# VinAIResearch/Counting-DETR

Hardware: AMD Instinct MI355X
Metric: images/sec FSCD-147 2nd-stage train step (higher is better)
Workload: dtype forward bf16x3 (fp32 operands split hi+lo, 3 bf16 MFMAs per product); data / weight gradients bf16 (both operands rounded to bf16, 1 MFMA per product); fp32 accumulate, fp32 storage, fp32 attention softmax / norms / losses / optimizer; 1 GPU; FSCD-147 2nd-stage train step (ResNet-50-DC5 + RCDA enc6/dec6, Q=300 learned, 800x800, T=[37, 120]), fwd+matcher+loss+bwd+clip+AdamW; images_per_gpu=2, global_batch=2, parallelism=dp1, graph=True, precision=bf16x3, precision_backward=bf16, frozen_stage_prefetch=True

## Files before the change

### counting_detr_amd/_ffi.py

```python
import ctypes as C
import os

import torch

_HERE = os.path.dirname(os.path.abspath(__file__))
LIB_PATH = os.environ.get("CDETR_LIB") or os.path.join(_HERE, "lib", "libcdetr_hip.so")

ROWS_DENSE, ROWS_CONV_FWD, ROWS_CONV_DGRAD = 0, 1, 2
_p = C.c_void_p


class ConvGeom(C.Structure):
    _fields_ = [("mode", C.c_int32), ("Ha", C.c_int32), ("Wa", C.c_int32), ("Hc", C.c_int32), ("Wc", C.c_int32),
                ("kh", C.c_int32), ("kw", C.c_int32), ("stride", C.c_int32), ("pad", C.c_int32), ("dil", C.c_int32)]


class GemmDesc(C.Structure):
    _fields_ = [("M", C.c_int32), ("N", C.c_int32), ("K", C.c_int32), ("taps", C.c_int32), ("batch", C.c_int32),
                ("b_layout", C.c_int32), ("relu", C.c_int32), ("precision", C.c_int32), ("out_scale", C.c_float),
                ("A", _p), ("lda", C.c_int64), ("sA", C.c_int64),
                ("B", _p), ("ldb", C.c_int64), ("sB", C.c_int64),
                ("C", _p), ("ldc", C.c_int64), ("sC", C.c_int64),
                ("w_scale", _p), ("bias", _p), ("resid", _p), ("ldr", C.c_int64), ("gate", _p), ("ldg", C.c_int64),
                ("g", ConvGeom), ("B_split", _p), ("batch_inner", C.c_int32), ("flags", C.c_int32),
# ... 1 lines not shown
                ("splitk_ws", _p), ("splitk_ws_bytes", C.c_int64), ("A16lo", _p), ("B16", _p), ("gate16", _p), ("C16lo", _p)]


class WgradDesc(C.Structure):
    _fields_ = [("P", C.c_int32), ("Nout", C.c_int32), ("Cin", C.c_int32), ("taps", C.c_int32), ("batch", C.c_int32), ("precision", C.c_int32),
                ("dY", _p), ("ldy", C.c_int64), ("sY", C.c_int64),
                ("X", _p), ("ldx", C.c_int64), ("sX", C.c_int64),
                ("dW", _p), ("ldw", C.c_int64), ("sW", C.c_int64),
                ("w_scale", _p), ("dbias", _p), ("g", ConvGeom), ("batch_inner", C.c_int32), ("wg_target", C.c_int32),
                ("sY2", C.c_int64), ("sX2", C.c_int64), ("sW2", C.c_int64), ("dY16", _p), ("X16", _p)]


class RcdaFwdDesc(C.Structure):
    _fields_ = [("N", C.c_int32), ("L", C.c_int32), ("H", C.c_int32), ("W", C.c_int32), ("nh", C.c_int32),
                ("precision", C.c_int32), ("scale", C.c_float), ("q_row", _p), ("q_col", _p), ("k_row", _p), ("k_col", _p), ("v", _p),
                ("mask_row", _p), ("mask_col", _p), ("out", _p), ("a_row", _p), ("a_col", _p), ("ws", _p), ("ws_bytes", C.c_int64)]


class RcdaBwdDesc(C.Structure):
    _fields_ = [("N", C.c_int32), ("L", C.c_int32), ("H", C.c_int32), ("W", C.c_int32), ("nh", C.c_int32),
                ("precision", C.c_int32), ("scale", C.c_float), ("d_out", _p), ("a_row", _p), ("a_col", _p), ("v", _p),
                ("ds_row", _p), ("ds_col", _p), ("d_v", _p), ("k_row", _p), ("k_col", _p), ("dq_row", _p), ("dq_col", _p),
                ("q_row", _p), ("q_col", _p), ("dk_row", _p), ("dk_col", _p)]


class AttnDesc(C.Structure):
    _fields_ = [("q", _p), ("k", _p), ("v", _p), ("ldq", C.c_int64), ("ldk", C.c_int64), ("ldv", C.c_int64), ("o", _p), ("lse", _p),
                ("d_o", _p), ("d_q", _p), ("d_k", _p), ("d_v", _p), ("ld_dq", C.c_int64), ("ld_dk", C.c_int64), ("ld_dv", C.c_int64),
                ("work", _p), ("N", C.c_int32), ("Lq", C.c_int32), ("Lk", C.c_int32), ("nh", C.c_int32), ("scale", C.c_float),
                ("precision", C.c_int32)]

# ... 208 lines not shown
```

### counting_detr_amd/csrc/common.h

```cpp
#pragma once
#include <hip/hip_runtime.h>
#include <stdint.h>

typedef float f32x16 __attribute__((ext_vector_type(16)));
typedef float f32x4 __attribute__((ext_vector_type(4)));
typedef __bf16 bf16x8 __attribute__((ext_vector_type(8)));

#define CDETR_OK 0
#define CDETR_ERR_ARG (-1)
#define CDETR_ERR_LAUNCH (-2)
#define CDETR_ERR_UNSUPPORTED (-3)

#include <stdlib.h>
static inline const char* cdetr_tune_env(const char* name) {
    static const bool tuning = getenv("CDETR_TUNING") != nullptr;
    return tuning ? getenv(name) : nullptr;
}

void cdetr_set_error(const char* fmt, ...);

#define CDETR_CHECK_ARG(cond, ...)          \
    do {                                    \
        if (!(cond)) {                      \
            cdetr_set_error(__VA_ARGS__);   \
// ... 57 lines not shown

__device__ __forceinline__ void stash_split4(__bf16* dst, int lo_off, float x0, float x1, float x2, float x3) {
    uint2 h, l;
    split_bf16_pk(x0, x1, h.x, l.x);
    split_bf16_pk(x2, x3, h.y, l.y);
    *reinterpret_cast<uint2*>(dst) = h;
    *reinterpret_cast<uint2*>(dst + lo_off) = l;
}
__device__ __forceinline__ void stash_hi4(__bf16* dst, float x0, float x1, float x2, float x3) {
    const f32x2 v0 = {x0, x1}, v1 = {x2, x3};
    uint2 h;
    h.x = __builtin_bit_cast(unsigned, __builtin_convertvector(v0, bf16x2));
    h.y = __builtin_bit_cast(unsigned, __builtin_convertvector(v1, bf16x2));
    *reinterpret_cast<uint2*>(dst) = h;
}
__device__ __forceinline__ f32x16 mfma_bf16x3(const bf16x8& ah, const bf16x8& al, const bf16x8& bh, const bf16x8& bl, f32x16 acc) {
    acc = __builtin_amdgcn_mfma_f32_32x32x16_bf16(al, bh, acc, 0, 0, 0);
    acc = __builtin_amdgcn_mfma_f32_32x32x16_bf16(ah, bl, acc, 0, 0, 0);
    acc = __builtin_amdgcn_mfma_f32_32x32x16_bf16(ah, bh, acc, 0, 0, 0);
    return acc;
}

template <int TERMS>
__device__ __forceinline__ f32x16 mfma_bf16_terms(const bf16x8& ah, const bf16x8& al, const bf16x8& bh, const bf16x8& bl, f32x16 acc) {
    if constexpr (TERMS == 1) return __builtin_amdgcn_mfma_f32_32x32x16_bf16(ah, bh, acc, 0, 0, 0);
    else return mfma_bf16x3(ah, al, bh, bl, acc);
}

template <int CTRL, int ROW_MASK>
__device__ __forceinline__ float dpp_pull(float x, float fill) {
// ... 21 lines not shown
```

### counting_detr_amd/csrc/igemm.hip

```cpp
#include "../../include/cdetr_hip.h"
#include "common.h"
#include "rows.h"
#include <stdlib.h>
#include <type_traits>
#include <vector>
#include <algorithm>

namespace {

constexpr int BK = 16;
constexpr int LDS_K = BK + 4;

__device__ __forceinline__ float4 ld4(const float* p) { return *reinterpret_cast<const float4*>(p); }
typedef unsigned u32x4 __attribute__((ext_vector_type(4)));
__device__ __forceinline__ u32x4 ld16(const __bf16* p) { return *reinterpret_cast<const u32x4*>(p); }
__device__ __forceinline__ float4 zero4() { return make_float4(0.f, 0.f, 0.f, 0.f); }

template <int BM, int BN, int BL>
__global__ __launch_bounds__(256) void igemm_kernel(const cdetr_gemm_desc d, const int tilesM, const int vecA,
                                                    const int vecB) {
    constexpr int FM = BM / 64, FN = BN / 64;
    constexpr int A_SLOTS = BM / 64, B_SLOTS = BN / 64;
    constexpr int LDS_N = BN + 4;
    constexpr int B_TILE = (BL == 0) ? BN * LDS_K : BK * LDS_N;
// ... 187 lines not shown
            for (int r = 0; r < 16; ++r) { rv[r] = 0.f; gv[r] = 1.f; }
            if (d.resid) {
#pragma unroll
                for (int r = 0; r < 16; ++r) rv[r] = d.resid[(long)min(mbase + (r & 3) + 8 * (r >> 2), d.M - 1) * d.ldr + nc];
            }
            if (d.gate) {
#pragma unroll
                for (int r = 0; r < 16; ++r) gv[r] = d.gate[(long)min(mbase + (r & 3) + 8 * (r >> 2), d.M - 1) * d.ldg + nc];
            }
#pragma unroll
            for (int r = 0; r < 16; ++r) {
                const int m = mbase + (r & 3) + 8 * (r >> 2);
                float v = (acc[a][b][r] + bias) * d.out_scale + rv[r];
                v = gv[r] > 0.f ? v : 0.f;
                if (d.relu) v = fmaxf(v, 0.f);
                if (nvalid && m < d.M) { C[(long)m * d.ldc + n] = v; if (C16) C16[(long)m * d.ldc + n] = (__bf16)v; }
            }
        }
    }
}

template <int BI, int BJ>
__global__ __launch_bounds__(256) void wgrad_kernel(const cdetr_wgrad_desc d, const int tilesI, const int tilesJ,
                                                    const int kt_per_slice) {
    constexpr int FM = BI / 64, FN = BJ / 64;
    constexpr int A_SLOTS = BI / 64, B_SLOTS = BJ / 64;
    constexpr int LDI = BI + 4, LDJ = BJ + 4;
    __shared__ __attribute__((aligned(16))) float smem[2 * BK * LDI + 2 * BK * LDJ];
    float* As = smem;
    float* Bs = smem + 2 * BK * LDI;

// ... 804 lines not shown
        float* red = smem;
#pragma unroll
        for (int s = 0; s < A_SLOTS; ++s) *reinterpret_cast<float4*>(red + kr * BI + cq + 32 * s) = bsum[s];
        __syncthreads();
        for (int i = tid; i < BI; i += 256) {
            float t = 0.f;
#pragma unroll 8
            for (int r = 0; r < 32; ++r) t += red[r * BI + i];
            if (i0 + i < d.Nout) atomicAdd(dbias + i0 + i, t);
        }
    }
}



typedef short s16x4 __attribute__((ext_vector_type(4)));
typedef short s16x8 __attribute__((ext_vector_type(8)));
__device__ __forceinline__ bf16x8 lds_tr8(const __bf16* p0, const __bf16* p1) {
    const s16x4 a = __builtin_amdgcn_ds_read_tr16_b64_v4i16((__attribute__((address_space(3))) s16x4*)(p0));
    const s16x4 b = __builtin_amdgcn_ds_read_tr16_b64_v4i16((__attribute__((address_space(3))) s16x4*)(p1));
    const s16x8 c = __builtin_shufflevector(a, b, 0, 1, 2, 3, 4, 5, 6, 7);
    return __builtin_bit_cast(bf16x8, c);
}

template <int BI, int BJ, int TERMS = 3>
__device__ __forceinline__ void wgrad_tr_body(const cdetr_wgrad_desc& d, const int tilesI, const int tilesJ, const int kt_per_slice,
                                              float* __restrict__ dbias, const int bx, const int by, const int bz, const bool single) {
    constexpr int BKF = 32;
    constexpr int FM = BI / 64, FN = BJ / 64;
    constexpr int A_SLOTS = BI / 32, B_SLOTS = BJ / 32;
    constexpr int BLK = 32 * 32;
    constexpr int PLANE_A = A_SLOTS * BLK, PLANE_B = B_SLOTS * BLK;
    constexpr int BUF = 2 * (PLANE_A + PLANE_B);
    extern __shared__ __attribute__((aligned(16))) float smem[];
    __bf16* Zs = reinterpret_cast<__bf16*>(smem);

    const int tid = threadIdx.x;
    const int lane = tid & 63, wid = tid >> 6;
// ... 507 lines not shown
#pragma unroll
    for (int r = 0; r < 4; ++r) red[wid][r * 64 + lane] = acc[r];
    __syncthreads();
    if (wid != 0) return;
    const int no = tn * 16 + i;
    if (no >= d.N) return;
#pragma unroll
    for (int r = 0; r < 4; ++r) {
        const int mo = tm * 16 + g4 * 4 + r;
        if (mo >= d.M) continue;
        const float sum = (red[0][r * 64 + lane] + red[1][r * 64 + lane]) + (red[2][r * 64 + lane] + red[3][r * 64 + lane]);
        float v = (sum + bias) * d.out_scale + rv[r];
        v = gv[r] > 0.f ? v : 0.f;
        if (d.relu) v = fmaxf(v, 0.f);
        C[(long)mo * d.ldc + no] = v;
        if (C16) C16[(long)mo * d.ldc + no] = (__bf16)v;
    }
}

template <int BL, int UB>
__global__ __launch_bounds__(256) void igemm_direct_kernel(const cdetr_gemm_desc d, const int tilesM, const int tilesN,
                                                           const int vecA, const int vecB) {
    igemm_direct_body<BL, UB>(d, tilesM, tilesN, vecA, vecB, blockIdx.x, blockIdx.z);
}

template <int BL, int UB>
__global__ __launch_bounds__(256) void igemm_direct_group_kernel(const GemmGroupArgs g) {
    int p = 0;
    while (p + 1 < g.n && (int)blockIdx.x >= g.blk0[p + 1]) ++p;
    const GemmGroupItem& it = g.it[p];
    const int lb = blockIdx.x - g.blk0[p];
// ... 760 lines not shown
```

### counting_detr_amd/csrc/rcda.hip

```cpp
#include "../../include/cdetr_hip.h"
#include "common.h"
#include <algorithm>
#include <type_traits>
#include <stdlib.h>

namespace {

__device__ __forceinline__ void xcd_slab(int& bx, int& by) {
    const int gx = gridDim.x, total = gx * gridDim.y;
    if (total & 7) return;
    const int lin = by * gx + bx;
    const int l2 = (lin & 7) * (total >> 3) + (lin >> 3);
    by = l2 / gx;
    bx = l2 - by * gx;
}


constexpr int D = 32;
constexpr int QW = 32;

__device__ __forceinline__ float4 ld4(const float* p) { return *reinterpret_cast<const float4*>(p); }

struct FwdSmem {
    int sw, sh;
// ... 400 lines not shown
        stamp(2 + side);
    }
    __syncthreads();
    stamp(4);

    {
        const int nq = min(QW, L - qbase);
        if (nq > 0 && save && d.a_row != nullptr) {
            save_rows(Srow, sm.sw, d.a_row + (((long)n * d.nh + head) * L + qbase) * Wp, nq, Wp, lane);
            save_rows(Scol, sm.sh, d.a_col + (((long)n * d.nh + head) * L + qbase) * Hp, nq, Hp, lane);
        }
    }
    stamp(5);
}

struct Fwd2Smem { int off_v, vts, total; };
__host__ __device__ inline Fwd2Smem fwd2_smem(const FwdSmem& sm, int H, int W, int KS) {
    Fwd2Smem s;
    s.off_v = sm.off_k;
    s.vts = 32 * KS + 8;
    const int vfloats = 2 * 32 * s.vts / 2;
    const int kfloats = (W + H) * KSTR;
    s.total = sm.off_k + (kfloats > vfloats ? kfloats : vfloats);
    return s;
}

template <int NW, int KS, int TH = 2, bool PROBE = false>
__global__ __launch_bounds__(64 * NW) void rcda_fwd2_kernel(const cdetr_rcda_fwd_desc d) {
    unsigned long long pt[5] = {0, 0, 0, 0, 0}, pacc[3] = {0, 0, 0};
    auto now = [&]() __attribute__((always_inline)) -> unsigned long long {
        if constexpr (PROBE) { const unsigned long long t = __builtin_amdgcn_s_memtime(); asm volatile("s_waitcnt lgkmcnt(0)" ::: "memory"); return t; }
        return 0ull;
    };
    pt[0] = now();
    constexpr int NT = 64 * NW, QB = QW * NW;
    constexpr int PD = 4;
    constexpr int NBLK = 16 * 4 * KS;
    constexpr int VB = (NBLK + NT - 1) / NT;
    constexpr int VTS = 32 * KS + 8;
    extern __shared__ __attribute__((aligned(16))) float smem[];
    const int H = d.H, W = d.W, L = d.L, E = d.nh * D;
    const FwdSmem sm = fwd_smem(H, W, NW);
    const int tid = threadIdx.x, lane = tid & 63, wid = tid >> 6;
// ... 61 lines not shown
    for (int s = 0; s < KS; ++s) {
        float x[8];
#pragma unroll
        for (int j = 0; j < 8; ++j) {
            const int w = 16 * s + 8 * g + j;
            x[j] = (w < W) ? Srow[i32 * sm.sw + w] : 0.f;
        }
        split_bf16x8(x, bh[s], bl[s]);
    }

    float outT[16];
#pragma unroll
    for (int r = 0; r < 16; ++r) outT[r] = 0.f;
    const f32x16 zero = {0.f, 0.f, 0.f, 0.f, 0.f, 0.f, 0.f, 0.f, 0.f, 0.f, 0.f, 0.f, 0.f, 0.f, 0.f, 0.f};

    vfetch(rv[0]); vfetch(rv[1]); vfetch(rv[2]); vfetch(rv[3]);
    vstash(rv[0], 0);
    __syncthreads();
    pt[2] = now();
    auto step = [&](auto U, int h) __attribute__((always_inline)) {
        constexpr int u = decltype(U)::value;
        const unsigned long long s0 = now();
        vfetch(rv[u]);
        const unsigned long long s1 = now();
        const float acolh = (h < he) ? Scol[i32 * sm.sh + h] : 0.f;
        const __bf16* vt = VT + (u & 1) * 32 * VTS + i32 * VTS + 8 * g;
        f32x16 T = zero;
#pragma unroll
        for (int s = 0; s < KS; ++s) {
            const bf16x8 ah = *reinterpret_cast<const bf16x8*>(vt + 16 * s);
// ... 5 lines not shown
        unsigned long long s2 = 0;
        if constexpr (PROBE) { asm volatile("" :: "v"(outT[0]), "v"(outT[15])); s2 = now(); }
        vstash(rv[(u + 1) % PD], (u + 1) & 1);
        const unsigned long long s3 = now();
        __syncthreads();
        if constexpr (PROBE) {
            const unsigned long long s4 = now();
            pacc[0] += s4 - s3; pacc[1] += s2 - s1; pacc[2] += (s1 - s0) + (s3 - s2);
        }
    };
    for (int h0 = hb; h0 < he; h0 += PD) {
        step(std::integral_constant<int, 0>{}, h0);
        step(std::integral_constant<int, 1>{}, h0 + 1);
        step(std::integral_constant<int, 2>{}, h0 + 2);
        step(std::integral_constant<int, 3>{}, h0 + 3);
    }
    pt[3] = now();
    if (hs > 1) {
        int* cnt = reinterpret_cast<int*>(d.ws);
        float* wsp = reinterpret_cast<float*>(cnt + RCDA_WS_COUNTERS);
        const int tile = blockIdx.y * gridDim.x + blockIdx.x;
        float* mine = wsp + ((long)tile * hs + hz) * 16 * NT + tid;
#pragma unroll
        for (int r = 0; r < 16; ++r) __hip_atomic_store(mine + r * NT, outT[r], __ATOMIC_RELAXED, __HIP_MEMORY_SCOPE_AGENT);
        __builtin_amdgcn_s_waitcnt(0);
        __syncthreads();
        int* flag = reinterpret_cast<int*>(smem + sm.off_k);
        if (tid == 0) {
            const int old = __hip_atomic_fetch_add(cnt + tile, 1, __ATOMIC_RELAXED, __HIP_MEMORY_SCOPE_AGENT);
            const int last = (old == hs - 1) ? 1 : 0;
// ... 849 lines not shown
}
inline int rcda_probe() {
    const char* p = cdetr_tune_env("CDETR_RCDA_PROBE");
    return p ? atoi(p) : 0;
}

}

extern "C" int cdetr_rcda_fwd(const cdetr_rcda_fwd_desc* dp, void* stream) {
    CDETR_CHECK_ARG(dp != nullptr, "cdetr_rcda_fwd: null descriptor");
    const cdetr_rcda_fwd_desc d = *dp;
    CDETR_CHECK_ARG(d.N > 0 && d.L > 0 && d.H > 0 && d.W > 0 && d.nh > 0, "cdetr_rcda_fwd: bad sizes");
    CDETR_CHECK_ARG(d.H <= 128 && d.W <= 1024, "cdetr_rcda_fwd: H must be <= 128 (got %d)", d.H);
    CDETR_CHECK_ARG(d.q_row && d.q_col && d.k_row && d.k_col && d.v && d.out, "cdetr_rcda_fwd: null pointer");
    CDETR_CHECK_ARG((d.a_row != nullptr) == (d.a_col != nullptr), "cdetr_rcda_fwd: a_row and a_col are saved together or not at all (both NULL: inference)");
    hipStream_t st = reinterpret_cast<hipStream_t>(stream);
    if (d.precision == 1 && d.W <= 96) {
        const int ks = (d.W + 15) / 16;
        auto go = [&](auto kern, int NWv, int KSv = 0, bool sliced = true) -> int {
            const FwdSmem sm = fwd_smem(d.H, d.W, NWv);
            const int bytes = fwd2_smem(sm, d.H, d.W, KSv ? KSv : ks).total * 4;
            int rc;
            if ((rc = set_smem(kern, bytes, "cdetr_rcda_fwd"))) return rc;
            dim3 grid((d.L + QW * NWv - 1) / (QW * NWv), d.N * d.nh), block(64 * NWv);
            if (sliced) grid.z = fwd2_slices(d, (int)(grid.x * grid.y), 64 * NWv, bytes);
            hipLaunchKernelGGL(kern, grid, block, bytes, st, d);
            return cdetr_launch_status("cdetr_rcda_fwd");
        };
        if (const int probe = rcda_probe(); probe && d.ws && ks == 4 && d.H <= 64)
            return probe == 5 ? go(rcda_fwd2_kernel<5, 4, 2, true>, 5, 0, false) : go(rcda_fwd2_kernel<4, 4, 2, true>, 4, 0, false);
        if (ks == 4 && rcda_wg5(d.L, d.N * d.nh)) return go(rcda_fwd2_kernel<5, 4>, 5);
        if (ks > 4 || d.H > 64) {
            if (d.H > 64 && d.H <= 96) return ks <= 4 ? go(rcda_fwd2_kernel<4, 4, 3>, 4, 4) : go(rcda_fwd2_kernel<4, 6, 3>, 4, 6);
            if (ks <= 4) return go(rcda_fwd2_kernel<4, 4>, 4, 4);
            return ks == 5 ? go(rcda_fwd2_kernel<4, 5>, 4) : go(rcda_fwd2_kernel<4, 6>, 4);
        }
        if (ks == 1) return go(rcda_fwd2_kernel<4, 1>, 4);
        if (ks == 2) return go(rcda_fwd2_kernel<4, 2>, 4);
        if (ks == 3) return go(rcda_fwd2_kernel<4, 3>, 4);
        return go(rcda_fwd2_kernel<4, 4>, 4);
    }
    if (d.H <= 32) return launch_rcda_fwd<1>(d, st);
    if (d.H <= 64) return launch_rcda_fwd<2>(d, st);
    return launch_rcda_fwd<4>(d, st);
}
// ... 81 lines not shown
```

### counting_detr_amd/ops.py

```python
import os

import torch

from . import _ffi
from ._ffi import CriterionDesc, MirrorItem, ConvGeom, GemmDesc, RcdaBwdDesc, RcdaFwdDesc, WgradDesc, check, lib, ptr, stream_ptr

import ctypes as C


PROFILE = None

import os as _os
PRECISION = int(_os.environ.get("CDETR_PRECISION", "1"))
PRECISION_BWD = int(_os.environ.get("CDETR_PRECISION_BWD", "3"))
MHA_BWD_BF16 = _os.environ.get("CDETR_MHA_BWD_BF16", "0") == "1"


def bwd_precision():
    return PRECISION_BWD if PRECISION == 1 else PRECISION


class arithmetic:

    def __init__(self, precision, precision_bwd=None):
        self.want = (int(precision), int(PRECISION_BWD if precision_bwd is None else precision_bwd))

    def __enter__(self):
        global PRECISION, PRECISION_BWD
        self.saved = (PRECISION, PRECISION_BWD)
        PRECISION, PRECISION_BWD = self.want
        return self

    def __exit__(self, *exc):
        global PRECISION, PRECISION_BWD
        PRECISION, PRECISION_BWD = self.saved
        return False


class scope:
    _KEYS = ("MIRROR", "BRANCH_BESIDE", "WGRAD_EVERY", "AFTER_BACKBONE", "WG_DEFER_NESTED", "ZERO_ARENA", "RCDA_SAVE", "PROFILE")

    def __init__(self, **kw):
        assert all(k in self._KEYS for k in kw), kw
        self.want = kw

    def __enter__(self):
        g = globals()
        self.saved = {k: g[k] for k in self.want}
        g.update(self.want)
        return self

    def __exit__(self, *exc):
        globals().update(self.saved)
        return False

# ... 443 lines not shown
            return hit
        r = self._find(self.f_entries, self._fb, w, scale)
        if r is None:
            out = None
        else:
            (base, nbytes, off, R, Cc, taps, sptr, _), row0 = r
            out = self.flat_fs[off + row0 * Cc * taps:]
        self._memo_f[key] = out
        return out


AFTER_BACKBONE = None
MIRROR = None


def linear_fwd(x2d, weight, bias=None, relu=False, resid=None, out_scale=1.0, out=None):
    M, K = x2d.shape
    N = weight.shape[0]
    y = out if out is not None else torch.empty((M, N), device=x2d.device, dtype=torch.float32)
    sp = MIRROR.lookup_fwd(weight) if MIRROR is not None else None
    gemm_raw(x2d, x2d.stride(0), weight, weight.stride(0), y, y.stride(0), M, N, K, bias=bias, relu=relu,
             resid=resid, ldr=(resid.stride(0) if resid is not None else 0), out_scale=out_scale, B_split=sp)
    return y


def linear_dgrad(dy2d, weight, gate=None, resid=None, dy16=None, twin=False):
    M, N = dy2d.shape
    K = weight.shape[1]
    dx = torch.empty((M, K), device=dy2d.device, dtype=torch.float32)
    m = MIRROR.lookup(weight) if MIRROR is not None else None
    if m is not None:
        dx16 = torch.empty((M, K), device=dy2d.device, dtype=torch.bfloat16) if twin else None
        gemm_raw(dy2d, dy2d.stride(0), m[0], m[1], dx, K, M, K, N, b_layout=0,
                 gate=gate, ldg=(gate.stride(0) if gate is not None else 0),
                 resid=resid, ldr=(resid.stride(0) if resid is not None else 0), B_split=m[2], B16=m[3], precision=bwd_precision(),
                 A16=dy16, C16=dx16)
        return (dx, dx16) if twin else dx
    gemm_raw(dy2d, dy2d.stride(0), weight, weight.stride(0), dx, K, M, K, N, b_layout=1,
# ... 409 lines not shown
    Nb, H, W, Cc = x.shape
    Ho, Wo = (H - 1) // 2 + 1, (W - 1) // 2 + 1
    y = torch.empty((Nb, Ho, Wo, Cc), device=x.device, dtype=torch.float32)
    if split:
        yh = torch.empty((Nb, Ho, Wo, Cc), device=x.device, dtype=torch.bfloat16)
        yl = torch.empty((Nb, Ho, Wo, Cc), device=x.device, dtype=torch.bfloat16)
        check(lib().cdetr_maxpool3x3s2_split(ptr(x), ptr(y), ptr(yh), ptr(yl), Nb, H, W, Cc, stream_ptr()), "cdetr_maxpool3x3s2_split")
        return y, yh, yl
    check(lib().cdetr_maxpool3x3s2(ptr(x), ptr(y), Nb, H, W, Cc, stream_ptr()), "cdetr_maxpool3x3s2")
    return y


RCDA_SKIP_SAVE = os.environ.get("CDETR_RCDA_SKIP_SAVE", "1") != "0"
RCDA_SAVE = True
RCDA_SLICES = os.environ.get("CDETR_RCDA_SLICES", "1") != "0"
FUSE_RCDA_DQ = os.environ.get("CDETR_RCDA_FUSE_DQ", "1") != "0"
FUSE_RCDA_DK = os.environ.get("CDETR_RCDA_FUSE_DK", "1") != "0"


def rcda_pads(H, W):
    return (H + 7) & ~7, (W + 3) & ~3


def rcda_fwd_raw(q_row, q_col, k_row, k_col, v, mask_row, mask_col, nh, save=None):
    N, L, E = q_row.shape
    H, W = v.shape[1:3]
    assert E == nh * 32, "the RCDA kernels are specialised for head_dim 32"
    Hp, Wp = rcda_pads(H, W)
    if save is None:
        save = RCDA_SAVE or not RCDA_SKIP_SAVE
    out = torch.empty((N, L, E), device=v.device, dtype=torch.float32)
    a_row = torch.empty((N, nh, L, Wp), device=v.device, dtype=torch.float32) if save else None
    a_col = torch.empty((N, nh, L, Hp), device=v.device, dtype=torch.float32) if save else None
    d = RcdaFwdDesc()
    d.N, d.L, d.H, d.W, d.nh, d.scale = N, L, H, W, nh, 32 ** -0.5
    d.precision = PRECISION
    d.q_row, d.q_col, d.k_row, d.k_col, d.v = ptr(q_row), ptr(q_col), ptr(k_row), ptr(k_col), ptr(v)
    d.mask_row, d.mask_col = ptr(mask_row), ptr(mask_col)
    d.out, d.a_row, d.a_col = ptr(out), ptr(a_row), ptr(a_col)
    if RCDA_SLICES:
        d.ws, d.ws_bytes = ptr(splitk_ws()), SPLITK_BYTES
    fl = 2.0 * N * nh * L * (H * W * 32 + (H + W) * 32)
    with _Timed("rcda_fwd", fl, None,
                4.0 * N * (3 * L * E + (H + W) * E + H * W * E + nh * L * (Hp + Wp)), fl * _TERMS[d.precision]):
        check(lib().cdetr_rcda_fwd(C.byref(d), stream_ptr()), "cdetr_rcda_fwd")
    return out, a_row, a_col


def rcda_zero_numel(v, k_row, k_col):
    return v.numel() + k_row.numel() + k_col.numel()


def rcda_bwd_raw(d_out, q_row, q_col, k_row, k_col, v, a_row, a_col, nh, zbuf=None):
    N, L, E = q_row.shape
# ... 329 lines not shown
    N, H, W, Cc = T.shape
    out = torch.empty_like(T)
    check(lib().cdetr_bcast_add2(ptr(T), ptr(Br), ptr(Bc), ptr(out), N, H, W, Cc, sr, sc, stream_ptr()), "cdetr_bcast_add2")
    return out


def _wg(dy2d, x2d, wparam, bparam, lo, hi):
    if not wparam.requires_grad:
        return
    gw = grad_buffer(wparam)[lo:hi]
    gb = grad_buffer(bparam)[lo:hi] if (bparam is not None and bparam.requires_grad) else None
    wgrad_raw(dy2d, dy2d.stride(0), x2d, x2d.stride(0), gw, gw.stride(0), dy2d.shape[0], hi - lo, x2d.shape[1], dbias=gb,
              may_defer=True)


class EncoderLayerFn(torch.autograd.Function):

    @staticmethod
    def forward(ctx, src, posemb_row, posemb_col, mask_row, mask_col, layer, anchor):
        N, H, W, Cc = src.shape
        R = N * H * W
        att = layer.self_attn
        E, nh = att.embed_dim, att.num_heads
        Wi, bi = att.in_proj_weight.detach(), att.in_proj_bias.detach()
        X = src.contiguous()
        Prow, Pcol = posemb_row.contiguous(), posemb_col.contiguous()
        Qr, Qc, Kr, Kc = posadd2_hw_reduce(X, Prow, Pcol)
        with gemm_queue():
            q_row = linear_fwd(Qr.view(R, Cc), Wi[0:E], bi[0:E]).view(N, H * W, E)
            q_col = linear_fwd(Qc.view(R, Cc), Wi[E:2 * E], bi[E:2 * E]).view(N, H * W, E)
            k_row = linear_fwd(Kr.view(N * W, Cc), Wi[2 * E:3 * E], bi[2 * E:3 * E]).view(N, W, E)
            k_col = linear_fwd(Kc.view(N * H, Cc), Wi[3 * E:4 * E], bi[3 * E:4 * E]).view(N, H, E)
            v = linear_fwd(X.view(R, Cc), Wi[4 * E:5 * E], bi[4 * E:5 * E]).view(N, H, W, E)
        o, a_row, a_col = rcda_fwd_raw(q_row, q_col, k_row, k_col, v, mask_row, mask_col, nh)
        Y1 = linear_fwd(o.view(R, E), att.out_proj.weight.detach(), att.out_proj.bias.detach(), resid=X.view(R, Cc))
        X1, mu1, rs1 = ln_fwd_raw(Y1, layer.norm1.weight.detach(), layer.norm1.bias.detach(), layer.norm1.eps)
        f = layer.ffn
        Hd = linear_fwd(X1, f.linear1.weight.detach(), f.linear1.bias.detach(), relu=True)
        Y2 = linear_fwd(Hd, f.linear2.weight.detach(), f.linear2.bias.detach(), resid=X1)
        X2, mu2, rs2 = ln_fwd_raw(Y2, f.norm2.weight.detach(), f.norm2.bias.detach(), f.norm2.eps)
        ctx.save_for_backward(X, Qr, Qc, Kr, Kc, q_row, q_col, k_row, k_col, v, a_row, a_col, o, Y1, mu1, rs1, X1, Hd, Y2, mu2, rs2)
        ctx.layer, ctx.dims = layer, (N, H, W, Cc, E, nh)
        return X2.view(N, H, W, Cc)

    @staticmethod
    def backward(ctx, dX2):
        with wgrad_queue():
            return EncoderLayerFn._backward(ctx, dX2)

# ... 118 lines not shown
        mem2 = memory.view(N * H * W, E)
        ctx.own_means = krm is None
        if ctx.own_means:
            krm, kcm = hw_reduce(memory, memory, posemb_row.contiguous(), posemb_col.contiguous(), 1.0 / H, 1.0 / W)
        krm2, kcm2 = krm.contiguous().view(N * W, E), kcm.contiguous().view(N * H, E)
        outs = []
        saved = []
        x = tgt.view(M, E)
        mem_side = []
        with gemm_queue():
            for layer in layers:
                ca = layer.cross_attn
                Wc, bc = ca.in_proj_weight.detach(), ca.in_proj_bias.detach()
                mem_side.append((linear_fwd(krm2, Wc[2 * E:3 * E], bc[2 * E:3 * E]).view(N, W, E),
                                 linear_fwd(kcm2, Wc[3 * E:4 * E], bc[3 * E:4 * E]).view(N, H, E),
                                 linear_fwd(mem2, Wc[4 * E:5 * E], bc[4 * E:5 * E]).view(N, H, W, E)))
        a1_next = None
        for li, layer in enumerate(layers):
            sa, ca, f = layer.self_attn, layer.cross_attn, layer.ffn
            nh = sa.num_heads
            Ws, bs = sa.in_proj_weight.detach(), sa.in_proj_bias.detach()
            Wc, bc = ca.in_proj_weight.detach(), ca.in_proj_bias.detach()
            if a1_next is None:
                a1, _ = add2(x, qpos.view(M, E))
            else:
                a1 = a1_next
            with gemm_queue():
                qk = linear_fwd(a1, Ws[0:2 * E], bs[0:2 * E])
                vs = linear_fwd(x, Ws[2 * E:3 * E], bs[2 * E:3 * E])
            o1, lse = mha_fwd_raw(qk.view(N, L, 2 * E), vs.view(N, L, E), nh, lens)
            Y2 = linear_fwd(o1.view(M, E), sa.out_proj.weight.detach(), sa.out_proj.bias.detach(), resid=x)
            T1, mu2, rs2, qr_in, qc_in = ln_fwd_add_raw(Y2, layer.norm2.weight.detach(), layer.norm2.bias.detach(), layer.norm2.eps,
                                                        qx.view(M, E), qy.view(M, E))
            with gemm_queue():
                q_row = linear_fwd(qr_in, Wc[0:E], bc[0:E]).view(N, L, E)
                q_col = linear_fwd(qc_in, Wc[E:2 * E], bc[E:2 * E]).view(N, L, E)
            k_row, k_col, v = mem_side[li]
            o2, a_row, a_col = rcda_fwd_raw(q_row, q_col, k_row, k_col, v, mask_row, mask_col, ca.num_heads)
            Y1 = linear_fwd(o2.view(M, E), ca.out_proj.weight.detach(), ca.out_proj.bias.detach(), resid=T1)
            T2, mu1, rs1 = ln_fwd_raw(Y1, layer.norm1.weight.detach(), layer.norm1.bias.detach(), layer.norm1.eps)
            Hd = linear_fwd(T2, f.linear1.weight.detach(), f.linear1.bias.detach(), relu=True)
            Y3 = linear_fwd(Hd, f.linear2.weight.detach(), f.linear2.bias.detach(), resid=T2)
            if li + 1 < len(layers):
                out, mu3, rs3, a1_next, _ = ln_fwd_add_raw(Y3, f.norm2.weight.detach(), f.norm2.bias.detach(), f.norm2.eps, qpos.view(M, E))
            else:
                out, mu3, rs3 = ln_fwd_raw(Y3, f.norm2.weight.detach(), f.norm2.bias.detach(), f.norm2.eps)
            outs.append(out.view(N, L, E))
            saved.append((x, a1, qk, vs, o1, lse, Y2, mu2, rs2, T1, qr_in, qc_in, q_row, q_col, k_row, k_col, v, a_row, a_col, o2,
                          Y1, mu1, rs1, T2, Hd, Y3, mu3, rs3))
            x = out
        ctx.layers, ctx.saved, ctx.dims = layers, saved, (N, L, E, H, W)
        ctx.shared = (mem2, krm2, kcm2)
        ctx.set_materialize_grads(False)
# ... 601 lines not shown
```

### include/cdetr_hip.h

```cpp
#ifndef CDETR_HIP_H
#define CDETR_HIP_H
#include <stddef.h>
#include <stdint.h>

#ifdef __cplusplus
extern "C" {
#endif

#define CDETR_ABI_VERSION 2

#define CDETR_ROWS_DENSE 0
#define CDETR_ROWS_CONV_FWD 1
#define CDETR_ROWS_CONV_DGRAD 2

typedef struct {
    int32_t mode;
    int32_t Ha, Wa;
    int32_t Hc, Wc;
    int32_t kh, kw, stride, pad, dil;
} cdetr_conv_geom;

typedef struct {
    int32_t M, N, K, taps;
    int32_t batch;
// ... 114 lines not shown
int cdetr_weight_mirror(const cdetr_mirror_item* items_dev, int32_t n_items, int32_t total_tiles, void* stream);
int cdetr_weight_images(const cdetr_mirror_item* items_dev, int32_t n_items, int32_t total_blocks, void* stream);

int cdetr_maxpool3x3s2(const float* X, float* Y, int32_t Nimg, int32_t H, int32_t W, int32_t C, void* stream);
int cdetr_maxpool3x3s2_split(const float* X, float* Y, void* Y16, void* Y16lo, int32_t Nimg, int32_t H, int32_t W, int32_t C, void* stream);

typedef struct {
    int32_t N, L, H, W, nh;
    int32_t precision;
    float scale;
    const float* q_row; const float* q_col; const float* k_row; const float* k_col; const float* v;
    const uint8_t* mask_row; const uint8_t* mask_col;
    float* out; float* a_row; float* a_col;
    void* ws;
    int64_t ws_bytes;
} cdetr_rcda_fwd_desc;
int cdetr_rcda_fwd(const cdetr_rcda_fwd_desc* d, void* stream);

typedef struct {
    int32_t N, L, H, W, nh;
    int32_t precision;
    float scale;
    const float* d_out; const float* a_row; const float* a_col; const float* v;
    float* ds_row; float* ds_col; float* d_v;
    const float* k_row; const float* k_col;
    float* dq_row; float* dq_col;
    const float* q_row; const float* q_col;
    float* dk_row; float* dk_col;
} cdetr_rcda_bwd_desc;
int cdetr_rcda_bwd(const cdetr_rcda_bwd_desc* d, void* stream);
// ... 197 lines not shown
```

Before: 242.1 images/s.

## Emit bf16 hi/lo planes of V from projection epilogue and stream them in RCDA forward

The value-projection GEMM epilogue now also writes bf16 hi and lo planes of its output. The RCDA forward kernel gets a planes variant that streams those pre-split planes straight into LDS through a 4-deep global_load_lds ring, then reads them back with transposing LDS loads for the bf16x3 MFMAs. This removes the per-tile fp32 load, hi/lo split and register stash of V inside the attention kernel. The cost is two extra bf16 writes per V element in the GEMM, extra memory for the planes, and a larger shared-memory ring.

```diff
diff --git a/counting_detr_amd/_ffi.py b/counting_detr_amd/_ffi.py
--- a/counting_detr_amd/_ffi.py
+++ b/counting_detr_amd/_ffi.py
@@ -39,7 +39,8 @@
 class RcdaFwdDesc(C.Structure):
     _fields_ = [("N", C.c_int32), ("L", C.c_int32), ("H", C.c_int32), ("W", C.c_int32), ("nh", C.c_int32),
                 ("precision", C.c_int32), ("scale", C.c_float), ("q_row", _p), ("q_col", _p), ("k_row", _p), ("k_col", _p), ("v", _p),
-                ("mask_row", _p), ("mask_col", _p), ("out", _p), ("a_row", _p), ("a_col", _p), ("ws", _p), ("ws_bytes", C.c_int64)]
+                ("mask_row", _p), ("mask_col", _p), ("out", _p), ("a_row", _p), ("a_col", _p), ("ws", _p), ("ws_bytes", C.c_int64),
+                ("v16", _p), ("v16lo", _p)]
 
 
 class RcdaBwdDesc(C.Structure):
diff --git a/counting_detr_amd/csrc/common.h b/counting_detr_amd/csrc/common.h
--- a/counting_detr_amd/csrc/common.h
+++ b/counting_detr_amd/csrc/common.h
@@ -95,6 +95,14 @@
     h.y = __builtin_bit_cast(unsigned, __builtin_convertvector(v1, bf16x2));
     *reinterpret_cast<uint2*>(dst) = h;
 }
+typedef short s16x4 __attribute__((ext_vector_type(4)));
+typedef short s16x8 __attribute__((ext_vector_type(8)));
+__device__ __forceinline__ bf16x8 lds_tr8(const __bf16* p0, const __bf16* p1) {
+    const s16x4 a = __builtin_amdgcn_ds_read_tr16_b64_v4i16((__attribute__((address_space(3))) s16x4*)(p0));
+    const s16x4 b = __builtin_amdgcn_ds_read_tr16_b64_v4i16((__attribute__((address_space(3))) s16x4*)(p1));
+    const s16x8 c = __builtin_shufflevector(a, b, 0, 1, 2, 3, 4, 5, 6, 7);
+    return __builtin_bit_cast(bf16x8, c);
+}
 __device__ __forceinline__ f32x16 mfma_bf16x3(const bf16x8& ah, const bf16x8& al, const bf16x8& bh, const bf16x8& bl, f32x16 acc) {
     acc = __builtin_amdgcn_mfma_f32_32x32x16_bf16(al, bh, acc, 0, 0, 0);
     acc = __builtin_amdgcn_mfma_f32_32x32x16_bf16(ah, bl, acc, 0, 0, 0);
diff --git a/counting_detr_amd/csrc/igemm.hip b/counting_detr_amd/csrc/igemm.hip
--- a/counting_detr_amd/csrc/igemm.hip
+++ b/counting_detr_amd/csrc/igemm.hip
@@ -225,7 +225,14 @@
                 float v = (acc[a][b][r] + bias) * d.out_scale + rv[r];
                 v = gv[r] > 0.f ? v : 0.f;
                 if (d.relu) v = fmaxf(v, 0.f);
-                if (nvalid && m < d.M) { C[(long)m * d.ldc + n] = v; if (C16) C16[(long)m * d.ldc + n] = (__bf16)v; }
+                if (nvalid && m < d.M) {
+                    C[(long)m * d.ldc + n] = v;
+                    if (C16) {
+                        const __bf16 h = (__bf16)v;
+                        C16[(long)m * d.ldc + n] = h;
+                        if (C16lo) C16lo[(long)m * d.ldc + n] = (__bf16)(v - (float)h);
+                    }
+                }
             }
         }
     }
@@ -1060,14 +1067,6 @@
 
 
 
-typedef short s16x4 __attribute__((ext_vector_type(4)));
-typedef short s16x8 __attribute__((ext_vector_type(8)));
-__device__ __forceinline__ bf16x8 lds_tr8(const __bf16* p0, const __bf16* p1) {
-    const s16x4 a = __builtin_amdgcn_ds_read_tr16_b64_v4i16((__attribute__((address_space(3))) s16x4*)(p0));
-    const s16x4 b = __builtin_amdgcn_ds_read_tr16_b64_v4i16((__attribute__((address_space(3))) s16x4*)(p1));
-    const s16x8 c = __builtin_shufflevector(a, b, 0, 1, 2, 3, 4, 5, 6, 7);
-    return __builtin_bit_cast(bf16x8, c);
-}
 
 template <int BI, int BJ, int TERMS = 3>
 __device__ __forceinline__ void wgrad_tr_body(const cdetr_wgrad_desc& d, const int tilesI, const int tilesJ, const int kt_per_slice,
@@ -1605,7 +1604,11 @@
         v = gv[r] > 0.f ? v : 0.f;
         if (d.relu) v = fmaxf(v, 0.f);
         C[(long)mo * d.ldc + no] = v;
-        if (C16) C16[(long)mo * d.ldc + no] = (__bf16)v;
+        if (C16) {
+            const __bf16 h = (__bf16)v;
+            C16[(long)mo * d.ldc + no] = h;
+            if (C16lo) C16lo[(long)mo * d.ldc + no] = (__bf16)(v - (float)h);
+        }
     }
 }
 
diff --git a/counting_detr_amd/csrc/rcda.hip b/counting_detr_amd/csrc/rcda.hip
--- a/counting_detr_amd/csrc/rcda.hip
+++ b/counting_detr_amd/csrc/rcda.hip
@@ -1,5 +1,6 @@
 #include "../../include/cdetr_hip.h"
 #include "common.h"
+#include "dl_common.h"
 #include <algorithm>
 #include <type_traits>
 #include <stdlib.h>
@@ -438,19 +439,52 @@
     stamp(5);
 }
 
+template <int OFF>
+__device__ __forceinline__ s16x4 lds_tr4_asm(unsigned addr) {
+    s16x4 r;
+    asm volatile("ds_read_b64_tr_b16 %0, %1 offset:%2" : "=v"(r) : "v"(addr), "n"(OFF) : "memory");
+    return r;
+}
+template <int KS, int S = 0>
+__device__ __forceinline__ void tr_tile_issue(unsigned addr, s16x4 (&fr)[KS][4]) {
+    if constexpr (S < KS) {
+        fr[S][0] = lds_tr4_asm<1024 * S>(addr);
+        fr[S][1] = lds_tr4_asm<1024 * S + 256>(addr);
+        fr[S][2] = lds_tr4_asm<1024 * (KS + S)>(addr);
+        fr[S][3] = lds_tr4_asm<1024 * (KS + S) + 256>(addr);
+        tr_tile_issue<KS, S + 1>(addr, fr);
+    }
+}
+template <int KS, int S = 0>
+__device__ __forceinline__ f32x16 tr_tile_mfma(s16x4 (&fr)[KS][4], const bf16x8 (&bh)[KS], const bf16x8 (&bl)[KS], f32x16 T) {
+    if constexpr (S < KS) {
+        asm volatile("s_waitcnt lgkmcnt(%4)" : "+v"(fr[S][0]), "+v"(fr[S][1]), "+v"(fr[S][2]), "+v"(fr[S][3]) : "n"(4 * (KS - 1 - S)) : "memory");
+        const bf16x8 ah = __builtin_bit_cast(bf16x8, (s16x8)__builtin_shufflevector(fr[S][0], fr[S][1], 0, 1, 2, 3, 4, 5, 6, 7));
+        const bf16x8 al = __builtin_bit_cast(bf16x8, (s16x8)__builtin_shufflevector(fr[S][2], fr[S][3], 0, 1, 2, 3, 4, 5, 6, 7));
+        T = mfma_bf16x3(ah, al, bh[S], bl[S], T);
+        __builtin_amdgcn_sched_barrier(0);
+        return tr_tile_mfma<KS, S + 1>(fr, bh, bl, T);
+    } else {
+        return T;
+    }
+}
+
+constexpr int FWD2_RING = 4;
 struct Fwd2Smem { int off_v, vts, total; };
-__host__ __device__ inline Fwd2Smem fwd2_smem(const FwdSmem& sm, int H, int W, int KS) {
+__host__ __device__ inline Fwd2Smem fwd2_smem(const FwdSmem& sm, int H, int W, int KS, bool planes = false) {
     Fwd2Smem s;
     s.off_v = sm.off_k;
     s.vts = 32 * KS + 8;
-    const int vfloats = 2 * 32 * s.vts / 2;
+    const int vfloats = planes ? FWD2_RING * 2 * KS * 256
+                               : 2 * 32 * s.vts / 2;
     const int kfloats = (W + H) * KSTR;
     s.total = sm.off_k + (kfloats > vfloats ? kfloats : vfloats);
     return s;
 }
 
-template <int NW, int KS, int TH = 2, bool PROBE = false>
+template <int NW, int KS, int TH = 2, bool PROBE = false, bool PL = false>
 __global__ __launch_bounds__(64 * NW) void rcda_fwd2_kernel(const cdetr_rcda_fwd_desc d) {
+    static_assert(!PL || (!PROBE && KS <= 4 && TH == 2), "planes form: product kernels of maps up to 64 x 64");
     unsigned long long pt[5] = {0, 0, 0, 0, 0}, pacc[3] = {0, 0, 0};
     auto now = [&]() __attribute__((always_inline)) -> unsigned long long {
         if constexpr (PROBE) { const unsigned long long t = __builtin_amdgcn_s_memtime(); asm volatile("s_waitcnt lgkmcnt(0)" ::: "memory"); return t; }
@@ -542,6 +576,59 @@
     for (int r = 0; r < 16; ++r) outT[r] = 0.f;
     const f32x16 zero = {0.f, 0.f, 0.f, 0.f, 0.f, 0.f, 0.f, 0.f, 0.f, 0.f, 0.f, 0.f, 0.f, 0.f, 0.f, 0.f};
 
+    if constexpr (PL) {
+        constexpr int RB = FWD2_RING;
+        constexpr int TILE_B = 2 * KS * 1024;
+        constexpr int LPW = (2 * KS + NW - 1) / NW;
+        unsigned char* VR = reinterpret_cast<unsigned char*>(smem + sm.off_k);
+        const int widu = __builtin_amdgcn_readfirstlane(wid);
+        const unsigned char* psrc[LPW];
+        int pdst[LPW];
+#pragma unroll
+        for (int k = 0; k < LPW; ++k) {
+            const int c = min(widu * LPW + k, 2 * KS - 1);
+            const int pl = c >= KS ? 1 : 0, s = c - pl * KS;
+            const int w = min(16 * s + (lane >> 2), W - 1);
+            psrc[k] = reinterpret_cast<const unsigned char*>(pl ? d.v16lo : d.v16) +
+                      ((((long)n * H + min(hb, H - 1)) * W + w) * E + head * D + (lane & 3) * 8) * 2;
+            pdst[k] = c * 1024;
+        }
+        const long tileB = (long)W * E * 2;
+        int hfp = min(hb, H - 1);
+        auto pissue = [&](int slot) __attribute__((always_inline)) {
+#pragma unroll
+            for (int k = 0; k < LPW; ++k)
+                __builtin_amdgcn_global_load_lds((gbl_vp)psrc[k], (lds_vp)(VR + slot * TILE_B + pdst[k]), 16, 0, 0);
+            ++hfp;
+            if (hfp < H) {
+#pragma unroll
+                for (int k = 0; k < LPW; ++k) psrc[k] += tileB;
+            }
+        };
+        const int l16 = lane & 15;
+        const int toff = (8 * g + (l16 >> 2)) * 64 + (16 * (i32 >> 4) + 4 * (l16 & 3)) * 2;
+        const unsigned vr0 = (unsigned)(unsigned long)(lds_vp)VR + toff;
+#pragma unroll
+        for (int t = 0; t < RB - 1; ++t) pissue(t);
+        int st = 0, sn = RB - 1;
+        for (int h = hb; h < he; ++h) {
+            wait_vm(LPW * (RB - 2));
+            __builtin_amdgcn_s_barrier();
+            __builtin_amdgcn_sched_barrier(0);
+            pissue(sn);
+            const float acolh = Scol[i32 * sm.sh + h];
+            s16x4 fr[KS][4];
+            tr_tile_issue<KS>(vr0 + st * TILE_B, fr);
+            const f32x16 T = tr_tile_mfma<KS>(fr, bh, bl, zero);
+#pragma unroll
+            for (int r = 0; r < 16; ++r) outT[r] = fmaf(acolh, T[r], outT[r]);
+            __builtin_amdgcn_sched_barrier(0);
+            st = (st + 1 == RB) ? 0 : st + 1;
+            sn = (sn + 1 == RB) ? 0 : sn + 1;
+        }
+        wait_vm(0);
+    }
+    if constexpr (!PL) {
     vfetch(rv[0]); vfetch(rv[1]); vfetch(rv[2]); vfetch(rv[3]);
     vstash(rv[0], 0);
     __syncthreads();
@@ -577,6 +664,7 @@
         step(std::integral_constant<int, 1>{}, h0 + 1);
         step(std::integral_constant<int, 2>{}, h0 + 2);
         step(std::integral_constant<int, 3>{}, h0 + 3);
+    }
     }
     pt[3] = now();
     if (hs > 1) {
@@ -1456,12 +1544,16 @@
     CDETR_CHECK_ARG(d.H <= 128 && d.W <= 1024, "cdetr_rcda_fwd: H must be <= 128 (got %d)", d.H);
     CDETR_CHECK_ARG(d.q_row && d.q_col && d.k_row && d.k_col && d.v && d.out, "cdetr_rcda_fwd: null pointer");
     CDETR_CHECK_ARG((d.a_row != nullptr) == (d.a_col != nullptr), "cdetr_rcda_fwd: a_row and a_col are saved together or not at all (both NULL: inference)");
+    CDETR_CHECK_ARG((d.v16 != nullptr) == (d.v16lo != nullptr) && ((reinterpret_cast<uintptr_t>(d.v16) | reinterpret_cast<uintptr_t>(d.v16lo)) & 15) == 0,
+                    "cdetr_rcda_fwd: v16 and v16lo come together, 16-byte aligned");
     hipStream_t st = reinterpret_cast<hipStream_t>(stream);
     if (d.precision == 1 && d.W <= 96) {
         const int ks = (d.W + 15) / 16;
-        auto go = [&](auto kern, int NWv, int KSv = 0, bool sliced = true) -> int {
+        const char* pl_env = cdetr_tune_env("CDETR_RCDA_PLANES");
+        const bool planes = d.v16 && ks <= 4 && d.H <= 64 && !(pl_env && atoi(pl_env) == 0);
+        auto go = [&](auto kern, int NWv, int KSv = 0, bool sliced = true, bool pl = false) -> int {
             const FwdSmem sm = fwd_smem(d.H, d.W, NWv);
-            const int bytes = fwd2_smem(sm, d.H, d.W, KSv ? KSv : ks).total * 4;
+            const int bytes = fwd2_smem(sm, d.H, d.W, KSv ? KSv : ks, pl).total * 4;
             int rc;
             if ((rc = set_smem(kern, bytes, "cdetr_rcda_fwd"))) return rc;
             dim3 grid((d.L + QW * NWv - 1) / (QW * NWv), d.N * d.nh), block(64 * NWv);
@@ -1471,6 +1563,13 @@
         };
         if (const int probe = rcda_probe(); probe && d.ws && ks == 4 && d.H <= 64)
             return probe == 5 ? go(rcda_fwd2_kernel<5, 4, 2, true>, 5, 0, false) : go(rcda_fwd2_kernel<4, 4, 2, true>, 4, 0, false);
+        if (planes) {
+            if (ks == 4 && rcda_wg5(d.L, d.N * d.nh)) return go(rcda_fwd2_kernel<5, 4, 2, false, true>, 5, 0, true, true);
+            if (ks == 1) return go(rcda_fwd2_kernel<4, 1, 2, false, true>, 4, 0, true, true);
+            if (ks == 2) return go(rcda_fwd2_kernel<4, 2, 2, false, true>, 4, 0, true, true);
+            if (ks == 3) return go(rcda_fwd2_kernel<4, 3, 2, false, true>, 4, 0, true, true);
+            return go(rcda_fwd2_kernel<4, 4, 2, false, true>, 4, 0, true, true);
+        }
         if (ks == 4 && rcda_wg5(d.L, d.N * d.nh)) return go(rcda_fwd2_kernel<5, 4>, 5);
         if (ks > 4 || d.H > 64) {
             if (d.H > 64 && d.H <= 96) return ks <= 4 ? go(rcda_fwd2_kernel<4, 4, 3>, 4, 4) : go(rcda_fwd2_kernel<4, 6, 3>, 4, 6);
diff --git a/counting_detr_amd/ops.py b/counting_detr_amd/ops.py
--- a/counting_detr_amd/ops.py
+++ b/counting_detr_amd/ops.py
@@ -38,7 +38,7 @@
 
 
 class scope:
-    _KEYS = ("MIRROR", "BRANCH_BESIDE", "WGRAD_EVERY", "AFTER_BACKBONE", "WG_DEFER_NESTED", "ZERO_ARENA", "RCDA_SAVE", "PROFILE")
+    _KEYS = ("MIRROR", "BRANCH_BESIDE", "WGRAD_EVERY", "AFTER_BACKBONE", "WG_DEFER_NESTED", "ZERO_ARENA", "RCDA_SAVE", "PROFILE", "RCDA_PLANES")
 
     def __init__(self, **kw):
         assert all(k in self._KEYS for k in kw), kw
@@ -512,14 +512,17 @@
 MIRROR = None
 
 
-def linear_fwd(x2d, weight, bias=None, relu=False, resid=None, out_scale=1.0, out=None):
+def linear_fwd(x2d, weight, bias=None, relu=False, resid=None, out_scale=1.0, out=None, planes=False):
     M, K = x2d.shape
     N = weight.shape[0]
     y = out if out is not None else torch.empty((M, N), device=x2d.device, dtype=torch.float32)
     sp = MIRROR.lookup_fwd(weight) if MIRROR is not None else None
+    y16 = torch.empty((M, N), device=x2d.device, dtype=torch.bfloat16) if planes else None
+    ylo = torch.empty((M, N), device=x2d.device, dtype=torch.bfloat16) if planes else None
+    assert not planes or y.stride(0) == N, "the planes share the output's leading dimension"
     gemm_raw(x2d, x2d.stride(0), weight, weight.stride(0), y, y.stride(0), M, N, K, bias=bias, relu=relu,
-             resid=resid, ldr=(resid.stride(0) if resid is not None else 0), out_scale=out_scale, B_split=sp)
-    return y
+             resid=resid, ldr=(resid.stride(0) if resid is not None else 0), out_scale=out_scale, B_split=sp, C16=y16, C16lo=ylo)
+    return (y, y16, ylo) if planes else y
 
 
 def linear_dgrad(dy2d, weight, gate=None, resid=None, dy16=None, twin=False):
@@ -959,6 +962,7 @@
 RCDA_SKIP_SAVE = os.environ.get("CDETR_RCDA_SKIP_SAVE", "1") != "0"
 RCDA_SAVE = True
 RCDA_SLICES = os.environ.get("CDETR_RCDA_SLICES", "1") != "0"
+RCDA_PLANES = True
 FUSE_RCDA_DQ = os.environ.get("CDETR_RCDA_FUSE_DQ", "1") != "0"
 FUSE_RCDA_DK = os.environ.get("CDETR_RCDA_FUSE_DK", "1") != "0"
 
@@ -967,7 +971,7 @@
     return (H + 7) & ~7, (W + 3) & ~3
 
 
-def rcda_fwd_raw(q_row, q_col, k_row, k_col, v, mask_row, mask_col, nh, save=None):
+def rcda_fwd_raw(q_row, q_col, k_row, k_col, v, mask_row, mask_col, nh, save=None, v16=None, v16lo=None):
     N, L, E = q_row.shape
     H, W = v.shape[1:3]
     assert E == nh * 32, "the RCDA kernels are specialised for head_dim 32"
@@ -983,6 +987,9 @@
     d.q_row, d.q_col, d.k_row, d.k_col, d.v = ptr(q_row), ptr(q_col), ptr(k_row), ptr(k_col), ptr(v)
     d.mask_row, d.mask_col = ptr(mask_row), ptr(mask_col)
     d.out, d.a_row, d.a_col = ptr(out), ptr(a_row), ptr(a_col)
+    if v16 is not None and RCDA_PLANES:
+        assert v16.dtype == v16lo.dtype == torch.bfloat16 and v16.numel() == v16lo.numel() == v.numel() and v16.is_contiguous() and v16lo.is_contiguous()
+        d.v16, d.v16lo = ptr(v16), ptr(v16lo)
     if RCDA_SLICES:
         d.ws, d.ws_bytes = ptr(splitk_ws()), SPLITK_BYTES
     fl = 2.0 * N * nh * L * (H * W * 32 + (H + W) * 32)
@@ -1342,6 +1349,12 @@
               may_defer=True)
 
 
+def _value_proj(x2d, weight, bias):
+    if RCDA_PLANES and PRECISION == 1:
+        return linear_fwd(x2d, weight, bias, planes=True)
+    return linear_fwd(x2d, weight, bias), None, None
+
+
 class EncoderLayerFn(torch.autograd.Function):
 
     @staticmethod
@@ -1359,8 +1372,9 @@
             q_col = linear_fwd(Qc.view(R, Cc), Wi[E:2 * E], bi[E:2 * E]).view(N, H * W, E)
             k_row = linear_fwd(Kr.view(N * W, Cc), Wi[2 * E:3 * E], bi[2 * E:3 * E]).view(N, W, E)
             k_col = linear_fwd(Kc.view(N * H, Cc), Wi[3 * E:4 * E], bi[3 * E:4 * E]).view(N, H, E)
-            v = linear_fwd(X.view(R, Cc), Wi[4 * E:5 * E], bi[4 * E:5 * E]).view(N, H, W, E)
-        o, a_row, a_col = rcda_fwd_raw(q_row, q_col, k_row, k_col, v, mask_row, mask_col, nh)
+            v, v16, v16lo = _value_proj(X.view(R, Cc), Wi[4 * E:5 * E], bi[4 * E:5 * E])
+            v = v.view(N, H, W, E)
+        o, a_row, a_col = rcda_fwd_raw(q_row, q_col, k_row, k_col, v, mask_row, mask_col, nh, v16=v16, v16lo=v16lo)
         Y1 = linear_fwd(o.view(R, E), att.out_proj.weight.detach(), att.out_proj.bias.detach(), resid=X.view(R, Cc))
         X1, mu1, rs1 = ln_fwd_raw(Y1, layer.norm1.weight.detach(), layer.norm1.bias.detach(), layer.norm1.eps)
         f = layer.ffn
@@ -1509,7 +1523,7 @@
                 Wc, bc = ca.in_proj_weight.detach(), ca.in_proj_bias.detach()
                 mem_side.append((linear_fwd(krm2, Wc[2 * E:3 * E], bc[2 * E:3 * E]).view(N, W, E),
                                  linear_fwd(kcm2, Wc[3 * E:4 * E], bc[3 * E:4 * E]).view(N, H, E),
-                                 linear_fwd(mem2, Wc[4 * E:5 * E], bc[4 * E:5 * E]).view(N, H, W, E)))
+                                 _value_proj(mem2, Wc[4 * E:5 * E], bc[4 * E:5 * E])))
         a1_next = None
         for li, layer in enumerate(layers):
             sa, ca, f = layer.self_attn, layer.cross_attn, layer.ffn
@@ -1530,8 +1544,9 @@
             with gemm_queue():
                 q_row = linear_fwd(qr_in, Wc[0:E], bc[0:E]).view(N, L, E)
                 q_col = linear_fwd(qc_in, Wc[E:2 * E], bc[E:2 * E]).view(N, L, E)
-            k_row, k_col, v = mem_side[li]
-            o2, a_row, a_col = rcda_fwd_raw(q_row, q_col, k_row, k_col, v, mask_row, mask_col, ca.num_heads)
+            k_row, k_col, (v, v16, v16lo) = mem_side[li]
+            v = v.view(N, H, W, E)
+            o2, a_row, a_col = rcda_fwd_raw(q_row, q_col, k_row, k_col, v, mask_row, mask_col, ca.num_heads, v16=v16, v16lo=v16lo)
             Y1 = linear_fwd(o2.view(M, E), ca.out_proj.weight.detach(), ca.out_proj.bias.detach(), resid=T1)
             T2, mu1, rs1 = ln_fwd_raw(Y1, layer.norm1.weight.detach(), layer.norm1.bias.detach(), layer.norm1.eps)
             Hd = linear_fwd(T2, f.linear1.weight.detach(), f.linear1.bias.detach(), relu=True)
diff --git a/include/cdetr_hip.h b/include/cdetr_hip.h
--- a/include/cdetr_hip.h
+++ b/include/cdetr_hip.h
@@ -152,6 +152,8 @@
     float* out; float* a_row; float* a_col;
     void* ws;
     int64_t ws_bytes;
+    const void* v16;
+    const void* v16lo;
 } cdetr_rcda_fwd_desc;
 int cdetr_rcda_fwd(const cdetr_rcda_fwd_desc* d, void* stream);
 
```

After: 242.3 images/s, median of 2. No clear change (+0.1%).
